# tud-airlab/mppi-isaac

Measured on AMD Instinct MI355X. Metric: MPPI control-loop Hz (K samples x H horizon), Panda 7-DoF K=4096 H=20, higher is better.
Workload: dtype f32; 1 GPU; panda_stick reach (BASELINE configs[2]): ABA from URDF, no contact, fused reach cost; K_per_gpu=4096, K_total=4096, H=20, nu=7, substeps=2, closed_loop=True, parallelism=single GPU, noise=fixed halton-spline set, sampled once at construction (outside the loop)

## Files before the change

__graft_entry__.py:

```python
import glob
import json
import os
import subprocess
import sys

ROOT = os.path.dirname(os.path.abspath(__file__))
PKG = os.path.join(ROOT, "mppi-isaac_amd")
CSRC = os.path.join(PKG, "csrc")
for p in (PKG, ROOT):
    if p not in sys.path:
        sys.path.insert(0, p)

HIPCC_FLAGS = ["--offload-arch=gfx950", "-O3", "-std=c++17", "-fPIC", "-shared",
               "-fno-slp-vectorize"]
ILP_FLAGS = ["-mllvm", "-amdgpu-sched-strategy=" + os.environ.get("MPPI_EXPERIMENT_SCHED", "max-ilp")]
if os.environ.get("MPPI_EXPERIMENT_SLP"):
    HIPCC_FLAGS.remove("-fno-slp-vectorize")


DPP_LEAD_WAIT_FROM = 9

FORESTS = [("point_robot", "point_robot")]
MOVING_FORESTS = [("jackal", "jackal")]

# ... 92 lines not shown


def _variant_jobs(variant, units, headers):
    lib = os.path.join(CSRC, f"libmppi_hip{'_' + variant if variant else ''}.so")
    objdir = os.path.join(CSRC, "build" + ("_" + variant if variant else ""))
    os.makedirs(objdir, exist_ok=True)
    flags = [f for f in HIPCC_FLAGS if f != "-shared" and not (variant == "slp" and f == "-fno-slp-vectorize")] \
        + (["-DMPPI_SECTION_CLOCKS"] if variant == "sec" else []) \
        + ([f"-DMPPI_DUP={variant[3:]}"] if variant.startswith("dup") else []) \
        + ([f"-DMPPI_PAIR_SPLIT={variant[2:]}"] if variant.startswith("ps") else []) \
        + (["-DMPPI_HWID_DEBUG"] if variant == "hwid" else []) \
        + (["-DMPPI_NO_PARK"] if variant == "nopark" else []) \
        + (["-DMPPI_CHECK"] if variant == "check" else []) \
        + ([f"-D{variant[1:].upper()}"] if variant.startswith("x") else []) \
        + (ILP_FLAGS if variant == "ilp" else []) \
        + ([f"-DMPPI_SCENE_WAVES_PER_EU={variant[1:]}"] if variant.startswith("w") and variant[1:].isdigit() else [])
    jobs = []
    for src in units:
        obj = os.path.join(objdir, os.path.basename(src) + ".o")
        if _stale(obj, [src] + headers):
            free = os.path.basename(src).startswith("topo_") and not src.endswith("_scene.hip")
            scene_flags = ["-mllvm", "-amdgpu-sched-strategy=iterative-maxocc"] if (variant == "maxocc" and not free and src.endswith("_scene.hip")) else []
            if os.environ.get("MPPI_EXPERIMENT_SCENE_SCHED") and src.endswith("_scene.hip"):
                scene_flags = ["-mllvm", "-amdgpu-sched-strategy=" + os.environ["MPPI_EXPERIMENT_SCENE_SCHED"]]
            jobs.append((src, obj, flags + (ILP_FLAGS if free and variant != "noilp" else []) + scene_flags))
    objs = [os.path.join(objdir, os.path.basename(src) + ".o") for src in units]
    return jobs, objs, lib


def build() -> None:
    from concurrent.futures import ThreadPoolExecutor
    units = [os.path.join(CSRC, "mppi_hip.hip")] + generate_sources()
    variant = os.environ.get("MPPI_BUILD_VARIANT", "")
    headers = [os.path.join(CSRC, f) for f in ("mppi_kernels.hpp", "mppi_device.hpp", "mppi_quad.hpp", "mppi_oct.hpp", "mppi_scene.hpp", "mppi_scene_quad.hpp", "mppi_scene_oct.hpp", "mppi_pack.hpp",
                                               "topologies.inc", "topo_table.inc")]
    headers.append(os.path.join(ROOT, "include", "mppi_hip.h"))
    variants = [variant] + (["check"] if variant == "" and not os.environ.get("MPPI_SKIP_CHECK_BUILD") else [])
    plans = [_variant_jobs(v, units, headers) for v in variants]
    jobs = [j for p in plans for j in p[0]]
    with ThreadPoolExecutor(max_workers=min(len(jobs), os.cpu_count() or 1) or 1) as ex:
        list(ex.map(_compile, jobs))
    hipcc = os.environ.get("HIPCC", "/opt/rocm/bin/hipcc")
    for vjobs, objs, vlib in plans:
        if vjobs or _stale(vlib, objs):
            subprocess.run([hipcc, "--offload-arch=gfx950", "-shared", "-fPIC", "-o", vlib, *objs], check=True)
    lib = plans[0][2]
    subprocess.run(["make", "-C", os.path.join(ROOT, "oracle"), "-s"], check=True)
    import mppiisaac
    from mppiisaac.backend import capi
    import ctypes
    handle = ctypes.CDLL(lib)
    for sym in capi.EXPORTED_SYMBOLS:
        getattr(handle, sym)


def smoke() -> None:
    import numpy as np
    import torch

    from mppiisaac.objectives import PandaReachObjective
    from mppiisaac.planner.mppi_isaac import MPPIisaacPlanner
    from mppiisaac.utils.config_store import load_config
    from oracle.oracle import Oracle

    assert torch.cuda.is_available(), "smoke() needs a GPU"
    cfg = load_config({"defaults": [{"mppi": "panda"}, {"isaacgym": "normal"}], "actors": ["panda_stick", "goal"],
                       "initial_actor_positions": [[0.0, 0.0, 0.0]], "nx": 14},
# ... 25 lines not shown
```

mppi-isaac_amd/csrc/mppi_hip.hip:

```cpp
#include <atomic>
#include <chrono>
#include <cstring>
#include <fstream>
#include <mutex>
#include <sstream>
#include <unordered_set>

#include <dlfcn.h>
#include <fcntl.h>
#include <spawn.h>
#include <sys/stat.h>
#include <sys/wait.h>
#include <unistd.h>

#include "mppi_kernels.hpp"
#include "topo_table.inc"

namespace {

thread_local std::string g_err;

int fail(int code, const std::string &msg) {
    g_err = msg;
    return code;
// ... 190 lines not shown
std::string lib_dir() {
    Dl_info info;
    if (dladdr((void *)&mppi_create, &info) == 0 || !info.dli_fname) return "";
    std::string p = info.dli_fname;
    const size_t k = p.rfind('/');
    return k == std::string::npos ? "." : p.substr(0, k);
}
bool file_exists(const std::string &p) {
    struct stat st;
    return stat(p.c_str(), &st) == 0 && S_ISREG(st.st_mode);
}
bool mkdir_p(const std::string &dir) {
    for (size_t i = 1; i <= dir.size(); i++)
        if (i == dir.size() || dir[i] == '/') {
            const std::string d = dir.substr(0, i);
            if (mkdir(d.c_str(), i == dir.size() ? 0700 : 0755) != 0 && errno != EEXIST) return false;
        }
    return true;
}
bool owned_and_private(const std::string &path, bool is_dir, std::string &why) {
    struct stat st;
    if (stat(path.c_str(), &st) != 0) { why = path + ": " + std::strerror(errno); return false; }
    if (is_dir ? !S_ISDIR(st.st_mode) : !S_ISREG(st.st_mode)) { why = path + " is not a " + (is_dir ? "directory" : "regular file"); return false; }
    if (st.st_uid != geteuid()) { why = path + " belongs to uid " + std::to_string((long)st.st_uid) + ", this process runs as " + std::to_string((long)geteuid()); return false; }
    if (st.st_mode & (S_IWGRP | S_IWOTH)) {
        char m[8];
        std::snprintf(m, sizeof m, "%04o", (unsigned)(st.st_mode & 07777));
        why = path + " is writable by group or others (mode " + m + ")";
        return false;
    }
    return true;
}
bool source_key(const std::string &dir, uint64_t &key, std::string &err) {
    const char *files[] = {"mppi_kernels.hpp", "mppi_device.hpp", "mppi_quad.hpp", "mppi_oct.hpp", "mppi_scene.hpp", "mppi_scene_quad.hpp", "mppi_scene_oct.hpp",
                           "mppi_pack.hpp", "topologies.inc", "../../include/mppi_hip.h"};
    uint64_t h = 1469598103934665603ull;
    for (const char *f : files) {
        std::ifstream in(dir + "/" + f, std::ios::binary);
        if (!in) { err = "kernel sources not found next to the library (" + dir + "/" + f + ")"; return false; }
        char buf[1 << 16];
        while (in.read(buf, sizeof buf) || in.gcount() > 0) {
            for (std::streamsize i = 0; i < in.gcount(); i++) h = (h ^ (unsigned char)buf[i]) * 1099511628211ull;
            if (!in) break;
        }
    }
    for (const char *f : kJitFlags)
        for (const char *q = f; *q; q++) h = (h ^ (unsigned char)*q) * 1099511628211ull;
    key = h;
    return true;
}
std::string cache_dir() {
    if (const char *e = std::getenv("MPPI_JIT_CACHE")) return e;
    if (const char *e = std::getenv("XDG_CACHE_HOME")) return std::string(e) + "/mppi_hip";
    if (const char *e = std::getenv("HOME")) return std::string(e) + "/.cache/mppi_hip";
    return "/tmp/mppi_hip_" + std::to_string((long)getuid());
}
std::string find_hipcc() {
    if (const char *e = std::getenv("HIPCC")) return e;
    for (const char *p : {"/opt/rocm/bin/hipcc", "/usr/bin/hipcc", "/usr/local/bin/hipcc"})
        if (access(p, X_OK) == 0) return p;
    return "";
}
pid_t spawn_to_log(const std::vector<std::string> &argv, const std::string &log) {
    std::vector<char *> av;
    for (const std::string &a : argv) av.push_back(const_cast<char *>(a.c_str()));
    av.push_back(nullptr);
    posix_spawn_file_actions_t fa;
// ... 193 lines not shown
                                                      (c->hm.n_light_pairs != 0 ? (size_t)kLightFloats : 0));
            c->lds_bytes_table = sizeof(unsigned) * (size_t)scene_table_dwords(c->hm.n_shapes, c->hm.n_pairs);
            const char *mode = std::getenv("MPPI_ROLLOUT");
            c->quad = !(mode && std::string(mode) == "lane");
            if (c->hm.n_bases > 1) c->quad = false;
            const bool oct = c->quad && !(mode && std::string(mode) == "quad") && cfg->num_samples >= 8;
            c->lanes_per_sample = !c->quad ? 1 : (oct ? 8 : 4);
            c->launch_rollout = c->quad ? (oct ? e->rollout_scene_oct : e->rollout_scene_quad) : e->rollout_scene;
            c->helper_wave = oct && e->rollout_scene_pair != nullptr && !(mode && std::string(mode) == "oct") && c->hm.n_pairs <= kPairKernelMaxPairs &&
                             c->hm.n_light_pairs == 0;
            if (c->helper_wave) c->launch_rollout = e->rollout_scene_pair;
            if (oct) {
                c->launch_rollout_traj = e->rollout_scene_traj;
                c->launch_materialise_traj = e->materialise_scene_traj;
            }
            c->launch_sim_step = c->quad ? e->sim_step_scene_quad : e->sim_step_scene;
            c->step_feeds_back = c->quad;
            c->launch_materialise = e->materialise_scene;
            if (hipSetDevice(device) == hipSuccess) {
                c->lds_bytes_static = e->static_lds();
                if (c->lds_bytes_quad + c->lds_bytes_table + c->lds_bytes_static <= 160 * 1024)
                    lds_err = e->raise_lds(c->lds_bytes <= 160 * 1024 ? c->lds_bytes : 0, c->lds_bytes_quad + c->lds_bytes_table);
            }
        } else {
            const char *mode = std::getenv("MPPI_ROLLOUT");
            c->quad = !(mode && std::string(mode) == "lane");
            int cus = 256;
            (void)hipDeviceGetAttribute(&cus, hipDeviceAttributeMultiprocessorCount, device);
            (void)hipGetLastError();
            const bool oct_fits = (cfg->num_samples + 7) / 8 <= 4 * cus || (mode && std::string(mode) == "oct");
            const bool oct = c->quad && !(mode && std::string(mode) == "quad") && cfg->num_samples >= 8 && oct_fits;
            c->lanes_per_sample = c->quad ? (oct ? 8 : 4) : 1;
            c->launch_rollout = c->quad ? (oct ? e->rollout_oct : e->rollout_quad) : e->rollout;
            c->launch_rollout_lane = e->rollout;
            if (c->quad) {
                c->launch_rollout_traj = oct ? e->rollout_oct_traj : e->rollout_traj;
                c->launch_materialise_traj = e->materialise_traj;
                c->launch_materialise_traj_link = e->materialise_traj_link;
            }
            c->launch_combine_world = e->combine_world;
            const char *ws = std::getenv("MPPI_WORLD_STEP");
            const bool world_quad = cfg->num_samples == 1 && !(ws && std::string(ws) == "lane");
            c->launch_sim_step = (c->quad && (cfg->num_samples >= 64 || world_quad)) ? e->sim_step_quad : e->sim_step;
            c->launch_materialise = e->materialise;
        }
        break;
    }
    if (ok && ((c->quad ? 0 : c->lds_bytes) > 160 * 1024 || c->lds_bytes_quad + c->lds_bytes_table + c->lds_bytes_static > 160 * 1024)) {
        delete c;
        return fail(MPPI_EUNSUPPORTED, "contact scene needs more than 160 KiB of LDS per workgroup (dynamic rows + table + the kernels' static __shared__)");
    }
    if (ok && lds_err != hipSuccess) {
        std::string msg = std::string("hipFuncSetAttribute(MaxDynamicSharedMemorySize): ") + hipGetErrorString(lds_err);
        delete c;
        return fail(MPPI_EHIP, msg);
    }
    if (!ok) {
        std::string t = c->topo;
        delete c;
        return fail(MPPI_EUNSUPPORTED, "kinematic tree " + t + " is not instantiated in this library and could not be built on demand: " + jit_err);
    }
    hipError_t e = hipSetDevice(device);
    if (e != hipSuccess) {
        delete c;
        return fail(MPPI_EHIP, std::string("hipSetDevice: ") + hipGetErrorString(e));
    }
// ... 690 lines not shown
#endif
int mppi_set_profiling(mppi_ctx_t *c, int on) {
    CTX_TRY(c);
    c->profiling = on != 0;
    c->profile_period = on > 1 ? on : 1;
    for (int w = 0; w < 3; w++) c->ev_used[w] = c->ev_seen[w] = 0;
    if (on)
        for (int w = 0; w < 3; w++)
            while (c->ev[w].size() < 512) {
                hipEvent_t a, b;
                if (hipEventCreate(&a) != hipSuccess || hipEventCreate(&b) != hipSuccess) { (void)hipGetLastError(); break; }
                c->ev[w].emplace_back(a, b);
            }
    return MPPI_OK;
}
int mppi_kernel_ms(mppi_ctx_t *c, int which, float *ms) {
    CTX_TRY(c);
    if (which < 0 || which > 2 || !ms) return fail(MPPI_EINVAL, "bad argument");
    HIP_TRY(hipStreamSynchronize(c->stream));
    size_t n = c->ev_used[which];
    if (n == 0) return fail(MPPI_ESTATE, "no profiled launches recorded");
    double tot = 0;
    for (size_t i = 0; i < n; i++) {
        float t = 0;
        HIP_TRY(hipEventElapsedTime(&t, c->ev[which][i].first, c->ev[which][i].second));
        tot += t;
    }
    *ms = (float)(tot / n);
    c->ev_used[which] = 0;
    return MPPI_OK;
}
int mppi_kernel_info(mppi_ctx_t *c, char *buf, int buflen) {
    CTX_TRY(c);
    std::snprintf(buf, buflen, "topology=%s rollout=%s K=%d H=%d nu=%d waves=%d block=%d bytes_alg=%zu", c->topo.c_str(), c->scene ? (c->helper_wave ? "scene-oct-pair" : (c->lanes_per_sample == 8 ? "scene-oct" : (c->quad ? "scene-quad" : "scene"))) : (c->quad ? (c->lanes_per_sample == 8 ? "oct" : "quad") : "lane"), c->K, c->H, c->nu, c->quad ? c->n_quads * ((c->lanes_per_sample == 8 && !c->scene) ? 2 : 1) : c->n_waves, kWave,
                  (size_t)4 * (3 * (size_t)c->K * c->HN + 2 * (size_t)c->K + c->HN));
    return MPPI_OK;
}

}
```

mppi-isaac_amd/csrc/mppi_kernels.hpp:

```cpp
#pragma once
#include <hip/hip_runtime.h>

#include <cstddef>
#include <cstdio>
#include <cstdlib>
#include <cstring>
#include <string>
#include <vector>

#include "mppi_pack.hpp"
#include "mppi_scene.hpp"
#include "mppi_quad.hpp"
#include "mppi_oct.hpp"
#include "mppi_scene_quad.hpp"
#include "mppi_scene_oct.hpp"

using namespace mppi;

struct mppi_ctx;

namespace {

constexpr int kWave = 64;

__device__ __forceinline__ float wave_sum(float v) {
#pragma unroll
    for (int o = 32; o > 0; o >>= 1) v += __shfl_xor(v, o, kWave);
    return v;
}
__device__ __forceinline__ float wave_min(float v) {
#pragma unroll
    for (int o = 32; o > 0; o >>= 1) v = fminf(v, __shfl_xor(v, o, kWave));
    return v;
}

template <class T>
__global__ __launch_bounds__(kWave) void k_rollout(const DevModel *__restrict__ m, const DevCfg *__restrict__ cfg,
                                                   const DevCost *__restrict__ cost, const float *__restrict__ x0_dof,
                                                   const float *__restrict__ x0_root, const float *__restrict__ U,
                                                   const float *__restrict__ eps, const float *__restrict__ prior,
                                                   float *__restrict__ du, float *__restrict__ S, float *__restrict__ viz,
                                                   float *__restrict__ partials);

__device__ __forceinline__ void wave_record(CCfg &cfg, float s, bool live, const float *__restrict__ du, int k, float *__restrict__ rec) {
    const int K = cfg.K, HN = cfg.H * cfg.nu;
    const bool fin = live && isfinite(s);
    const float beta = wave_min(fin ? s : INFINITY);
    const float w = fin ? __expf(-(s - beta) * cfg.inv_lambda) : 0.f;
    const float eta = wave_sum(w);
    const int lane = threadIdx.x & (kWave - 1);
    if (lane == 0) {
        rec[0] = beta;
        rec[1] = eta;
    }
    const size_t kk = live ? (size_t)k : 0;
    int j = 0;
// ... 313 lines not shown
        s_lin = oct_lin_place((MPPI_LDS_AS void *)s_lin_raw, &lm.b[0]);
        if ((int)threadIdx.x < T::NB) {
            DevBody b = ((const DevModel *)m)->b[threadIdx.x];
            b.k1 = oct_lin_view(b.k1);
            s_lin[threadIdx.x] = b;
        }
    }
    __syncthreads();
    const int nb = gridDim.x;
    const int chunk = (nb % 16 == 0) ? (int)(blockIdx.x % 8) * (nb / 8) + (int)(blockIdx.x / 8) : (int)blockIdx.x;
    const int k = chunk * 16 + (LAY == 8 ? (int)(threadIdx.x >> 6) * 8 + oct_slot() : (int)(threadIdx.x >> 2));
    const int lane4 = threadIdx.x & 3;
    const bool live = k < cfg->K;
    const bool leader = lane4 == 0 && (LAY == 4 || oct_half() == 0);
    float s = INFINITY;
    if (live) {
        if constexpr (LAY == 8) {
            const OctAba ab{oct_bodies(&lm.b[0], s_lin), oct_lane()};
            if (((CModel *)m)->all_revolute) s = quad_rollout<T, 0, DUMP>(lm, *(CCfg *)cfg, *(CCost *)cost, sc, x0_dof, x0_root, eps, prior, du, viz, k, leader, quad_row(), lane4 < 3, traj, ab);
            else s = quad_rollout<T, -1, DUMP>(lm, *(CCfg *)cfg, *(CCost *)cost, sc, x0_dof, x0_root, eps, prior, du, viz, k, leader, quad_row(), lane4 < 3, traj, ab);
        } else {
            if (((CModel *)m)->all_revolute) s = quad_rollout<T, 0, DUMP>(lm, *(CCfg *)cfg, *(CCost *)cost, sc, x0_dof, x0_root, eps, prior, du, viz, k, leader, quad_row(), lane4 < 3, traj);
            else s = quad_rollout<T, -1, DUMP>(lm, *(CCfg *)cfg, *(CCost *)cost, sc, x0_dof, x0_root, eps, prior, du, viz, k, leader, quad_row(), lane4 < 3, traj);
        }
        if (leader) S[k] = s;
    }
    if constexpr (LAY == 8) {
        oct_record2(*(CCfg *)cfg, s, live && leader, du, chunk * 16, partials + (size_t)chunk * (2 + cfg->H * cfg->nu), oct_slot());
        fold_after_record<2>(*(CCfg *)cfg, partials, fold_ctr, fold_out);
    } else {
        quad_record(*(CCfg *)cfg, s, live && leader, du, chunk * 16, partials + (size_t)chunk * (2 + cfg->H * cfg->nu));
        fold_after_record(*(CCfg *)cfg, partials, fold_ctr, fold_out);
    }
    if (wave_clk != nullptr && threadIdx.x == 0) {
        wave_clk[2 * chunk] = clk0;
        wave_clk[2 * chunk + 1] = wall_clock64();
    }
#endif
}

constexpr int kCombineThreads = 1024;
constexpr int kCombineGroups = 8;
constexpr int kCombineWorldThreads = 512;
template <int NT>
__device__ __forceinline__ void combine_update(CCfg &cfg, const float *__restrict__ recs, int nrec, int mode, float *__restrict__ out,
                                               float *__restrict__ U, float *__restrict__ action, float *__restrict__ beta_eta, float *s_act,
                                               const float *__restrict__ filt) {
    __shared__ float s_red[NT];
    __shared__ float s_part[kCombineGroups][MPPI_MAX_H * MPPI_MAX_NU];
    constexpr int kMaxScale = 4096;
    __shared__ float s_scale[kMaxScale];
    const int HN = cfg.H * cfg.nu, RF = 2 + HN, nu = cfg.nu;
    const int tid = threadIdx.x;
    const int wid = tid >> 6, lane = tid & 63;
    const float U_old = (mode != 0 && tid < HN) ? U[tid] : 0.f;
    const bool mine = tid < nrec;
    const float er0 = mine ? recs[(size_t)tid * RF + 1] : 0.f, br0 = mine ? recs[(size_t)tid * RF] : 0.f;
    float b = er0 > 0.f ? br0 : INFINITY;
    for (int r = tid + NT; r < nrec; r += NT)
        if (recs[(size_t)r * RF + 1] > 0.f) b = fminf(b, recs[(size_t)r * RF]);
    b = wave_min(b);
    if (lane == 0) s_red[wid] = b;
    __syncthreads();
    float beta = s_red[lane & (NT / kWave - 1)];
#pragma unroll
    for (int o = NT / kWave / 2; o > 0; o >>= 1) beta = fminf(beta, __shfl_xor(beta, o, kWave));
// ... 991 lines not shown
    const int i = threadIdx.x;
    if (i < n) {
        x0_dof[2 * i] = wq[i];
        x0_dof[2 * i + 1] = wqd[i];
    }
}

}

constexpr int kIoCmd = 16, kIoCmdSlots = 64, kIoDof = kIoCmd + 16 * kIoCmdSlots, kIoDofFloats = 32;
static_assert(kIoDofFloats == kIoMirrorRoot, "mirror layout");
constexpr int kIoFloats = kIoDof + kIoDofFloats + 13 * MPPI_MAX_ACTORS + 12;

struct mppi_ctx {
    int device = 0;
    float *h_io = nullptr, *d_io = nullptr;
    int free_slots = 2;
    unsigned io_cmd_next = 0, io_mirror_seq = 0;
    bool mirror_armed = false;
    hipStream_t stream = nullptr;
    mppi_model_t model;
    mppi_config_t cfg;
    DevModel hm;
    DevCfg hc;
    DevCost hk;
    int n = 0, A = 0, B = 0, K = 0, H = 0, nu = 0, HN = 0, RF = 0, n_waves = 0;
    int n_quads = 0;
    int lanes_per_sample = 1;
    float *d_traj = nullptr;
    DevCost *d_cost_none = nullptr;
    void (*launch_rollout_traj)(mppi_ctx *) = nullptr;
    void (*launch_materialise_traj)(mppi_ctx *, float *, float *, float *, float *) = nullptr;
    void (*launch_materialise_traj_link)(mppi_ctx *, int, float *) = nullptr;
    bool helper_wave = false;
    int n_partials = 0;
    bool quad = false;
    DevModel *d_model = nullptr;
    DevCfg *d_cfg = nullptr;
    DevCost *d_cost = nullptr;
    float *d_x0_dof = nullptr, *d_x0_root = nullptr, *d_U = nullptr, *d_eps = nullptr, *d_du = nullptr, *d_S = nullptr;
    float *d_prior = nullptr, *d_viz = nullptr, *d_partials = nullptr, *d_record = nullptr, *d_action = nullptr, *d_beta_eta = nullptr;
    float *d_q = nullptr, *d_qd = nullptr, *d_ctrl = nullptr;
    float *d_base = nullptr, *d_fr = nullptr, *d_cf = nullptr;
    float *d_filter = nullptr;
    float *h_action = nullptr;
    unsigned *d_seq = nullptr;
    unsigned seq_expected = 0;
    bool use_filter = false;
    bool scene = false;
    size_t lds_bytes = 0, lds_bytes_quad = 0;
    size_t lds_bytes_table = 0;
    size_t lds_bytes_static = 0;
    double *d_basis = nullptr, *d_sigma = nullptr;
    const float *eps_in = nullptr;
    bool has_prior = false, has_cost = false, profiling = false;
    bool partials_valid = false;
    bool fold = false;
    unsigned *d_fold_ctr = nullptr;
    float *d_fold = nullptr, *fold_out = nullptr;
    const float *recs_cur = nullptr;
    unsigned long long *d_wave_clk = nullptr;
    bool wave_clk_on = false;
    std::vector<std::pair<hipEvent_t, hipEvent_t>> ev[3];
    size_t ev_used[3] = {0, 0, 0}, ev_seen[3] = {0, 0, 0};
    int profile_period = 1;
    void (*launch_rollout)(mppi_ctx *) = nullptr;
    void (*launch_rollout_lane)(mppi_ctx *) = nullptr;
    bool prog_lane = false;
    void (*launch_sim_step)(mppi_ctx *, int, int, const float *) = nullptr;
    void (*launch_materialise)(mppi_ctx *, float *, float *, float *, float *) = nullptr;
    void (*launch_combine_world)(mppi_ctx *, const float *, int, mppi_ctx *) = nullptr;
    void (*launch_eval_cost)(mppi_ctx *, int, const float *, const float *, const float *, const float *, float *) = nullptr;
    std::string topo;
    float *fb_dof = nullptr, *fb_root = nullptr;
    bool step_feeds_back = false;
    void *d_inbox = nullptr;
    void **d_peers = nullptr;
    std::vector<void *> h_peers, ipc_opened;
    int mb_rank = -1, mb_n = 0, mb_nrec = 0;
    unsigned *d_mb_seq = nullptr, *d_mb_status = nullptr;
    float *d_gathered = nullptr, *d_own_rec = nullptr;
    size_t inbox_bytes = 0;
    bool peers_dirty = false;
    bool inbox_fine = false;
};

namespace mppi {
struct TopoEntry {
    int nb;
    int parents[MPPI_MAX_BODIES];
    size_t scene_lds_floats;
    int free_slots;
    void (*rollout)(mppi_ctx *);
    void (*rollout_quad)(mppi_ctx *);
    void (*rollout_oct)(mppi_ctx *);
    void (*rollout_oct_traj)(mppi_ctx *);
    void (*rollout_scene)(mppi_ctx *);
    void (*rollout_scene_quad)(mppi_ctx *);
    void (*rollout_scene_oct)(mppi_ctx *);
    void (*rollout_scene_pair)(mppi_ctx *);
    void (*rollout_traj)(mppi_ctx *);
    void (*rollout_scene_traj)(mppi_ctx *);
    void (*materialise_traj)(mppi_ctx *, float *, float *, float *, float *);
    void (*materialise_traj_link)(mppi_ctx *, int, float *);
    void (*materialise_scene_traj)(mppi_ctx *, float *, float *, float *, float *);
    void (*sim_step)(mppi_ctx *, int, int, const float *);
    void (*sim_step_quad)(mppi_ctx *, int, int, const float *);
    void (*sim_step_scene)(mppi_ctx *, int, int, const float *);
    void (*sim_step_scene_quad)(mppi_ctx *, int, int, const float *);
    void (*materialise)(mppi_ctx *, float *, float *, float *, float *);
    void (*materialise_scene)(mppi_ctx *, float *, float *, float *, float *);
    void (*combine_world)(mppi_ctx *, const float *, int, mppi_ctx *);
    void (*eval_cost)(mppi_ctx *, int, const float *, const float *, const float *, const float *, float *);
    hipError_t (*raise_lds)(size_t, size_t);
    size_t (*static_lds)();
};
}

namespace {

template <class T>
void launch_rollout_scene_t(mppi_ctx *c) {
    hipLaunchKernelGGL(k_rollout_scene<T>, dim3(c->n_waves), dim3(kWave), c->lds_bytes, c->stream, c->d_model, c->d_cfg, c->d_cost, c->d_x0_dof,
                       c->d_x0_root, c->d_U, c->eps_in, c->has_prior ? c->d_prior : nullptr, c->d_du, c->d_S, c->cfg.want_rollouts ? c->d_viz : nullptr,
                       c->d_partials);
}
template <class T>
constexpr bool kHasOctSolve = (T::NB > 4);
inline bool scene_oct_solve(const mppi_ctx *c) {
// ... 106 lines not shown
    auto ask = [&](const void *f) {
        hipFuncAttributes a;
        if (hipFuncGetAttributes(&a, f) == hipSuccess && a.sharedSizeBytes > mx) mx = a.sharedSizeBytes;
        else (void)hipGetLastError();
    };
    ask(reinterpret_cast<const void *>(&k_rollout_scene_quad<T, 4>));
    ask(reinterpret_cast<const void *>(&k_rollout_scene_quad<T, 8>));
    ask(reinterpret_cast<const void *>(&k_rollout_scene_quad<T, 8, 1, true>));
    if constexpr (kHasOctSolve<T>) {
        ask(reinterpret_cast<const void *>(&k_rollout_scene_quad<T, 8, 1, false, true>));
        ask(reinterpret_cast<const void *>(&k_rollout_scene_quad<T, 8, 1, true, true>));
    }
    if constexpr (T::NB <= 4) {
        ask(reinterpret_cast<const void *>(&k_rollout_scene_quad<T, 8, 2>));
        ask(reinterpret_cast<const void *>(&k_rollout_scene_quad<T, 8, 2, true>));
    }
    ask(reinterpret_cast<const void *>(&k_sim_step_scene_quad<T>));
    return mx;
}

template <class T>
void launch_rollout_quad_t(mppi_ctx *c) {
    hipLaunchKernelGGL(k_rollout_quad<T>, dim3(c->n_quads), dim3(kWave), 0, c->stream, c->d_model, c->d_cfg, c->d_cost, c->d_x0_dof, c->d_x0_root,
                       c->d_U, c->eps_in, c->has_prior ? c->d_prior : nullptr, c->d_du, c->d_S, c->cfg.want_rollouts ? c->d_viz : nullptr, c->d_partials,
                       c->fold ? c->d_fold_ctr : nullptr, c->fold_out, c->wave_clk_on ? c->d_wave_clk : nullptr);
}
template <class T>
void launch_rollout_oct_t(mppi_ctx *c) {
    hipLaunchKernelGGL((k_rollout_quad<T, false, 8>), dim3(c->n_quads), dim3(2 * kWave), 0, c->stream, c->d_model, c->d_cfg, c->d_cost, c->d_x0_dof, c->d_x0_root,
                       c->d_U, c->eps_in, c->has_prior ? c->d_prior : nullptr, c->d_du, c->d_S, c->cfg.want_rollouts ? c->d_viz : nullptr, c->d_partials,
                       c->fold ? c->d_fold_ctr : nullptr, c->fold_out, c->wave_clk_on ? c->d_wave_clk : nullptr);
}
template <class T>
void launch_rollout_oct_traj_t(mppi_ctx *c) {
    hipLaunchKernelGGL((k_rollout_quad<T, true, 8>), dim3(c->n_quads), dim3(2 * kWave), 0, c->stream, c->d_model, c->d_cfg, c->d_cost_none, c->d_x0_dof, c->d_x0_root,
                       c->d_U, c->eps_in, c->has_prior ? c->d_prior : nullptr, c->d_du, c->d_S, (float *)nullptr, c->d_partials,
                       (unsigned *)nullptr, c->fold_out, (unsigned long long *)nullptr, c->d_traj);
}
template <class T>
void launch_rollout_traj_t(mppi_ctx *c) {
    hipLaunchKernelGGL((k_rollout_quad<T, true>), dim3(c->n_quads), dim3(kWave), 0, c->stream, c->d_model, c->d_cfg, c->d_cost_none, c->d_x0_dof, c->d_x0_root,
                       c->d_U, c->eps_in, c->has_prior ? c->d_prior : nullptr, c->d_du, c->d_S, (float *)nullptr, c->d_partials,
                       (unsigned *)nullptr, c->fold_out, (unsigned long long *)nullptr, c->d_traj);
}
template <class T>
void launch_materialise_traj_t(mppi_ctx *c, float *dof, float *root, float *rb, float *cf) {
    const size_t HK = (size_t)c->H * c->K;
    hipLaunchKernelGGL(k_materialise<T>, dim3((unsigned)((HK + kWave - 1) / kWave)), dim3(kWave), 0, c->stream, c->d_model, (int)HK, c->d_x0_root, c->d_traj,
                       c->d_traj + (size_t)T::NB * HK, dof, root, rb, cf);
}
template <class T>
void launch_materialise_traj_link_t(mppi_ctx *c, int link, float *out) {
    const size_t HK = (size_t)c->H * c->K;
    hipLaunchKernelGGL(k_materialise_link<T>, dim3((unsigned)((HK + kWave - 1) / kWave)), dim3(kWave), 0, c->stream, c->d_model, (int)HK, c->d_x0_root, c->d_traj,
                       c->d_traj + (size_t)T::NB * HK, link, out);
}
template <class T>
void launch_combine_world_t(mppi_ctx *p, const float *recs, int n, mppi_ctx *w) {
    MailboxArgs mb;
    if (recs == nullptr) {
        mb.wave_recs = p->recs_cur; mb.n_wave = p->n_partials; mb.own = p->d_own_rec; mb.RF = p->RF; mb.rank = p->mb_rank; mb.n = p->mb_n;
        mb.peers = (void *const *)p->d_peers; mb.seq_ctr = p->d_mb_seq; mb.inbox = p->d_inbox; mb.gathered = p->d_gathered; mb.status = p->d_mb_status;
        mb.max_ticks = 200000000ull;
    }
    hipLaunchKernelGGL(k_combine_world<T>, dim3(1), dim3(kCombineWorldThreads), 0, p->stream, p->d_cfg, recs, n, p->d_U, p->d_action, p->d_beta_eta,
                       w->d_model, w->d_x0_root, w->d_q, w->d_qd, p->d_x0_dof, p->use_filter ? p->d_filter : nullptr, mb);
// ... 1 lines not shown
template <class T>
void launch_eval_cost_t(mppi_ctx *c, int n, const float *dof, const float *root, const float *rb, const float *cf, float *out) {
    hipLaunchKernelGGL(k_eval_cost<T>, dim3((n + kWave - 1) / kWave), dim3(kWave), 0, c->stream, c->d_model, c->d_cost, n, dof, root, rb, cf, out);
}
template <class T>
void launch_rollout_t(mppi_ctx *c) {
    hipLaunchKernelGGL(k_rollout<T>, dim3(c->n_waves), dim3(kWave), 0, c->stream, c->d_model, c->d_cfg, c->d_cost, c->d_x0_dof, c->d_x0_root,
                       c->d_U, c->eps_in, c->has_prior ? c->d_prior : nullptr, c->d_du, c->d_S, c->cfg.want_rollouts ? c->d_viz : nullptr, c->d_partials);
}
template <class T>
void launch_sim_step_t(mppi_ctx *c, int mode, int t, const float *u_ext) {
    hipLaunchKernelGGL(k_sim_step<T>, dim3(c->n_waves), dim3(kWave), 0, c->stream, c->d_model, c->d_cfg, mode, t, u_ext, c->d_x0_root, c->d_U,
                       c->eps_in, c->has_prior ? c->d_prior : nullptr, c->d_du, c->d_ctrl, c->d_q, c->d_qd);
}
template <class T>
void launch_sim_step_quad_t(mppi_ctx *c, int mode, int t, const float *u_ext) {
    hipLaunchKernelGGL(k_sim_step_quad<T>, dim3((c->K + 15) / 16), dim3(kWave), 0, c->stream, c->d_model, c->d_cfg, mode, t, u_ext, c->d_x0_root, c->d_U,
                       c->eps_in, c->has_prior ? c->d_prior : nullptr, c->d_du, c->d_ctrl, c->d_q, c->d_qd);
}
template <class T>
void launch_materialise_t(mppi_ctx *c, float *dof, float *root, float *rb, float *cf) {
    hipLaunchKernelGGL(k_materialise<T>, dim3(c->n_waves), dim3(kWave), 0, c->stream, c->d_model, c->K, c->d_x0_root, c->d_q, c->d_qd, dof, root,
                       rb, cf, c->mirror_armed ? c->d_io + kIoDof : nullptr, reinterpret_cast<unsigned *>(c->d_io), c->io_mirror_seq);
}

template <class T>
void fill_topo_entry_free(TopoEntry &e) {
    e.nb = T::NB;
    for (int i = 0; i < T::NB; i++) e.parents[i] = T::par[i];
    e.rollout = &launch_rollout_t<T>;
    e.rollout_quad = &launch_rollout_quad_t<T>;
    e.rollout_oct = &launch_rollout_oct_t<T>;
    e.rollout_oct_traj = &launch_rollout_oct_traj_t<T>;
    e.sim_step = &launch_sim_step_t<T>;
    e.sim_step_quad = &launch_sim_step_quad_t<T>;
    e.rollout_traj = &launch_rollout_traj_t<T>;
    e.materialise_traj = &launch_materialise_traj_t<T>;
    e.materialise_traj_link = &launch_materialise_traj_link_t<T>;
    e.materialise = &launch_materialise_t<T>;
    e.combine_world = &launch_combine_world_t<T>;
    e.eval_cost = &launch_eval_cost_t<T>;
}
template <class T>
void fill_topo_entry_scene(TopoEntry &e) {
    e.scene_lds_floats = (size_t)SceneLayout<T>::kCf;
    e.free_slots = kFreeSlots;
    e.rollout_scene = &launch_rollout_scene_t<T>;
    e.rollout_scene_quad = &launch_rollout_scene_quad_t<T, 4>;
    e.rollout_scene_oct = &launch_rollout_scene_quad_t<T, 8>;
    e.rollout_scene_pair = T::NB <= 4 ? &launch_rollout_scene_pair_t<T> : nullptr;
    e.sim_step_scene = &launch_sim_step_scene_t<T>;
    e.sim_step_scene_quad = &launch_sim_step_scene_quad_t<T>;
    e.rollout_scene_traj = &launch_rollout_scene_traj_t<T>;
    e.materialise_scene_traj = &launch_materialise_scene_traj_t<T>;
    e.materialise_scene = &launch_materialise_scene_t<T>;
    e.raise_lds = &raise_lds_limit<T>;
    e.static_lds = &static_lds_bytes_scene<T>;
}

}
```

mppi-isaac_amd/csrc/mppi_quad.hpp:

```cpp
#pragma once
#include <cstddef>

#include "mppi_device.hpp"

namespace mppi {

#if defined(__HIP_DEVICE_COMPILE__)
typedef float QF;
template <int CTRL>
__device__ __forceinline__ float quad_dpp(float x) {
    return __builtin_bit_cast(float, __builtin_amdgcn_mov_dpp(__builtin_bit_cast(int, x), CTRL, 0xf, 0xf, true));
}
__device__ __forceinline__ QF rot1(QF x) { return quad_dpp<0x49>(x); }
__device__ __forceinline__ QF rot2(QF x) { return quad_dpp<0x92>(x); }
template <int K>
__device__ __forceinline__ QF bc(QF x) { return quad_dpp<K * 0x55>(x); }
__device__ __forceinline__ int quad_row() { int l = threadIdx.x & 3; return l == 3 ? 0 : l; }
__device__ __forceinline__ QF qsel(float x0, float x1, float x2) { int r = quad_row(); return r == 0 ? x0 : (r == 1 ? x1 : x2); }
__device__ __forceinline__ QF qrep(float x) { return x; }
__device__ __forceinline__ float qlane0(QF x) { return x; }
__device__ __forceinline__ QF qsqrt(QF x) { return __builtin_amdgcn_sqrtf(x); }
__device__ __forceinline__ QF qrcp(QF x) { float r = __builtin_amdgcn_rcpf(x); return r * (2.f - x * r); }
__device__ __forceinline__ QF qabs(QF x) { return fabsf(x); }
__device__ __forceinline__ QF qclamp(QF v, QF lo, QF hi) { return __builtin_amdgcn_fmed3f(v, lo, hi); }
// ... 622 lines not shown
            {
                const QF lo = qrep(blk0[i].lower), hi = qrep(blk0[i].upper), z = qrep(0.f);
                const QF vlo = qclamp((lo - q[i]) * inv_h, qrep(-b.vmax), z), vhi = qclamp((hi - q[i]) * inv_h, z, qrep(b.vmax));
                v = qclamp(v, vlo, vhi);
                x = qclamp(q[i] + h * v, lo, hi);
            }
            q[i] = x;
            qd[i] = v;
        });
        quad_fk_from<T, JT>(blk0, q, P);
    }
}

template <class T, int JT, int LO, int HI>
MPPI_HD void quad_body_pose(const QPose<T, JT> &P, int body, QM3 &Rb, QF &pb) {
    if constexpr (HI - LO == 1) {
        if constexpr (LO < 0) {
            Rb = P.rot_base();
            pb = P.pos_base();
        } else {
            Rb = P.rot(LO);
            pb = P.pos(LO);
        }
#if defined(__HIP_DEVICE_COMPILE__)
        asm volatile("");
#endif
    } else {
        constexpr int MID = LO + (HI - LO) / 2;
        if (body < MID) quad_body_pose<T, JT, LO, MID>(P, body, Rb, pb);
        else quad_body_pose<T, JT, MID, HI>(P, body, Rb, pb);
    }
}

template <class T, class M, int JT>
MPPI_HD void quad_link_pose(M &m, const QPose<T, JT> &P, int l, QM3 &R, QF &p) {
    auto &L = m.l[l];
#if defined(__HIP_DEVICE_COMPILE__)
    const int body = __builtin_amdgcn_readfirstlane(L.body);
#else
    const int body = L.body;
#endif
    QM3 Rb;
    QF pb;
    quad_body_pose<T, JT, -1, T::NB>(P, body < 0 ? -1 : (body < T::NB ? body : T::NB - 1), Rb, pb);
    for (int c = 0; c < 3; c++) R.c[c] = Rb.c[0] * L.R[c] + Rb.c[1] * L.R[3 + c] + Rb.c[2] * L.R[6 + c];
    p = pb + Rb.c[0] * L.p[0] + Rb.c[1] * L.p[1] + Rb.c[2] * L.p[2];
}

struct StepConsts {
    CtrlBlock u_min, u_max, inv_sigma;
    float goal[4];
    float w[4];
    CtrlBlock Urow[MPPI_MAX_H];
};
#if defined(__HIP_DEVICE_COMPILE__)
typedef const MPPI_LDS_AS StepConsts LStep;
#else
typedef const StepConsts LStep;
#endif
MPPI_HD float step_const_entry(CCfg &cfg, CCost &c, const float *root, const float *U, int j) {
    constexpr int kU = (int)(offsetof(StepConsts, Urow) / sizeof(float));
    if (j < 16) return cfg.u_min.v[j];
    if (j < 32) return cfg.u_max.v[j - 16];
    if (j < 48) return cfg.inv_sigma.v[j - 32];
    if (j < 52) {
        const int a = c.actor[0], i = j - 48;
        if (i == 3) return 0.f;
        if (a >= 0) return root[13 * a + i];
        return i < 2 ? c.w[1 + i] : 0.f;
    }
    if (j < 56) return c.w[j - 52];
    const int t = (j - kU) >> 4, col = (j - kU) & 15;
    return (t < cfg.H && col < cfg.nu) ? U[t * cfg.nu + col] : 0.f;
}
MPPI_HD int step_const_count(CCfg &cfg) { return (int)(offsetof(StepConsts, Urow) / sizeof(float)) + cfg.H * 16; }

template <class T>
MPPI_HD QF quad_stage_cost(int kind, LStep &sc, const QF *q, const QM3 &R, QF p) {
    if (kind == kCostPointReach) {
// ... 139 lines not shown
```

Measured before the change: 8204 Hz (4096-sample x 20-step control iterations per second, summed over GPUs).

## Add oct-pair rollout splitting dynamics and control/cost work across wave pairs

Adds a new free-space rollout kernel in which each 256-thread block runs two owner waves that integrate dynamics and two helper waves that compute controls, noise application and stage costs. The two sides exchange per-step control rows and link poses through LDS with double-buffered slots and named barriers, and the weighted reduction is done over 16 samples per block. The host selects this kernel when the oct path applies, H<=32 and K/16 fits within the CU count. The aim is to take control and cost arithmetic off the critical dynamics path so it runs concurrently. In exchange it adds per-step barrier synchronisation and LDS traffic, and uses more waves per sample.

Result: faster. 9466 Hz (4096-sample x 20-step control iterations per second, summed over GPUs), median of 6 (+15.4%).

```diff
diff --git a/__graft_entry__.py b/__graft_entry__.py
--- a/__graft_entry__.py
+++ b/__graft_entry__.py
@@ -148,7 +148,7 @@
     from concurrent.futures import ThreadPoolExecutor
     units = [os.path.join(CSRC, "mppi_hip.hip")] + generate_sources()
     variant = os.environ.get("MPPI_BUILD_VARIANT", "")
-    headers = [os.path.join(CSRC, f) for f in ("mppi_kernels.hpp", "mppi_device.hpp", "mppi_quad.hpp", "mppi_oct.hpp", "mppi_scene.hpp", "mppi_scene_quad.hpp", "mppi_scene_oct.hpp", "mppi_pack.hpp",
+    headers = [os.path.join(CSRC, f) for f in ("mppi_kernels.hpp", "mppi_device.hpp", "mppi_quad.hpp", "mppi_oct.hpp", "mppi_oct_pair.hpp", "mppi_scene.hpp", "mppi_scene_quad.hpp", "mppi_scene_oct.hpp", "mppi_pack.hpp",
                                                "topologies.inc", "topo_table.inc")]
     headers.append(os.path.join(ROOT, "include", "mppi_hip.h"))
     variants = [variant] + (["check"] if variant == "" and not os.environ.get("MPPI_SKIP_CHECK_BUILD") else [])
diff --git a/mppi-isaac_amd/csrc/mppi_hip.hip b/mppi-isaac_amd/csrc/mppi_hip.hip
--- a/mppi-isaac_amd/csrc/mppi_hip.hip
+++ b/mppi-isaac_amd/csrc/mppi_hip.hip
@@ -246,7 +246,7 @@
     return true;
 }
 bool source_key(const std::string &dir, uint64_t &key, std::string &err) {
-    const char *files[] = {"mppi_kernels.hpp", "mppi_device.hpp", "mppi_quad.hpp", "mppi_oct.hpp", "mppi_scene.hpp", "mppi_scene_quad.hpp", "mppi_scene_oct.hpp",
+    const char *files[] = {"mppi_kernels.hpp", "mppi_device.hpp", "mppi_quad.hpp", "mppi_oct.hpp", "mppi_oct_pair.hpp", "mppi_scene.hpp", "mppi_scene_quad.hpp", "mppi_scene_oct.hpp",
                            "mppi_pack.hpp", "topologies.inc", "../../include/mppi_hip.h"};
     uint64_t h = 1469598103934665603ull;
     for (const char *f : files) {
@@ -506,6 +506,10 @@
             const bool oct = c->quad && !(mode && std::string(mode) == "quad") && cfg->num_samples >= 8 && oct_fits;
             c->lanes_per_sample = c->quad ? (oct ? 8 : 4) : 1;
             c->launch_rollout = c->quad ? (oct ? e->rollout_oct : e->rollout_quad) : e->rollout;
+            const bool pair_forced = mode && std::string(mode) == "oct-pair";
+            c->pair_free = oct && e->rollout_oct_pair != nullptr && !(mode && std::string(mode) == "oct") && cfg->horizon <= kPairTableH &&
+                           ((cfg->num_samples + 15) / 16 <= cus || pair_forced);
+            if (c->pair_free) c->launch_rollout = e->rollout_oct_pair;
             c->launch_rollout_lane = e->rollout;
             if (c->quad) {
                 c->launch_rollout_traj = oct ? e->rollout_oct_traj : e->rollout_traj;
@@ -1262,7 +1266,7 @@
 }
 int mppi_kernel_info(mppi_ctx_t *c, char *buf, int buflen) {
     CTX_TRY(c);
-    std::snprintf(buf, buflen, "topology=%s rollout=%s K=%d H=%d nu=%d waves=%d block=%d bytes_alg=%zu", c->topo.c_str(), c->scene ? (c->helper_wave ? "scene-oct-pair" : (c->lanes_per_sample == 8 ? "scene-oct" : (c->quad ? "scene-quad" : "scene"))) : (c->quad ? (c->lanes_per_sample == 8 ? "oct" : "quad") : "lane"), c->K, c->H, c->nu, c->quad ? c->n_quads * ((c->lanes_per_sample == 8 && !c->scene) ? 2 : 1) : c->n_waves, kWave,
+    std::snprintf(buf, buflen, "topology=%s rollout=%s K=%d H=%d nu=%d waves=%d block=%d bytes_alg=%zu", c->topo.c_str(), c->scene ? (c->helper_wave ? "scene-oct-pair" : (c->lanes_per_sample == 8 ? "scene-oct" : (c->quad ? "scene-quad" : "scene"))) : (c->quad ? (c->lanes_per_sample == 8 ? (c->pair_free ? "oct-pair" : "oct") : "quad") : "lane"), c->K, c->H, c->nu, c->quad ? c->n_quads * ((c->lanes_per_sample == 8 && !c->scene) ? (c->pair_free ? 4 : 2) : 1) : c->n_waves, kWave,
                   (size_t)4 * (3 * (size_t)c->K * c->HN + 2 * (size_t)c->K + c->HN));
     return MPPI_OK;
 }
diff --git a/mppi-isaac_amd/csrc/mppi_kernels.hpp b/mppi-isaac_amd/csrc/mppi_kernels.hpp
--- a/mppi-isaac_amd/csrc/mppi_kernels.hpp
+++ b/mppi-isaac_amd/csrc/mppi_kernels.hpp
@@ -12,6 +12,7 @@
 #include "mppi_scene.hpp"
 #include "mppi_quad.hpp"
 #include "mppi_oct.hpp"
+#include "mppi_oct_pair.hpp"
 #include "mppi_scene_quad.hpp"
 #include "mppi_scene_oct.hpp"
 
@@ -22,6 +23,7 @@
 namespace {
 
 constexpr int kWave = 64;
+constexpr int kPairTableH = 32;
 
 __device__ __forceinline__ float wave_sum(float v) {
 #pragma unroll
@@ -401,6 +403,152 @@
         quad_record(*(CCfg *)cfg, s, live && leader, du, chunk * 16, partials + (size_t)chunk * (2 + cfg->H * cfg->nu));
         fold_after_record(*(CCfg *)cfg, partials, fold_ctr, fold_out);
     }
+    if (wave_clk != nullptr && threadIdx.x == 0) {
+        wave_clk[2 * chunk] = clk0;
+        wave_clk[2 * chunk + 1] = wall_clock64();
+    }
+#endif
+}
+
+#if defined(__HIP_DEVICE_COMPILE__)
+template <class T>
+__device__ __forceinline__ void oct_record_pair(CCfg &cfg, LStep &sc, float s, bool live_leader, bool helper, const MPPI_LDS_AS float *utab, int k0,
+                                                float *__restrict__ rec, int slot) {
+    constexpr int NT = 4 * kWave, SPG = 16, kStride = PairLayout<T>::kStride, kRow = PairLayout<T>::kRow;
+    __shared__ float s_w[SPG], s_b[2], s_e[2];
+    const int K = cfg.K, nu = cfg.nu, HN = cfg.H * nu;
+    const int lane = threadIdx.x & (kWave - 1), wv = (threadIdx.x >> 6) & 1;
+    const bool fin = live_leader && isfinite(s);
+    const float bw = wave_min(fin ? s : INFINITY);
+    if (helper && lane == 0) s_b[wv] = bw;
+    MPPI_BARRIER(12);
+    const float beta = fminf(s_b[0], s_b[1]);
+    const float w = fin ? __expf(-(s - beta) * cfg.inv_lambda) : 0.f;
+    const float ew = wave_sum(w);
+    if (helper && lane == 0) s_e[wv] = ew;
+    if (helper && (lane & 3) == 0 && ((lane >> 3) & 1) == 0) s_w[wv * 8 + slot] = w;
+    MPPI_BARRIER(13);
+    if (threadIdx.x == 0) {
+        rec[0] = beta;
+        rec[1] = s_e[0] + s_e[1];
+    }
+    const int nlive = K - k0 < SPG ? K - k0 : SPG;
+    if (nlive == SPG && (K & 3) == 0) {
+        constexpr int kTrips = 2, NR = 2 * kWave;
+        if (threadIdx.x >= NR) return;
+        float wq[SPG];
+#pragma unroll
+        for (int q = 0; q < SPG; q++) wq[q] = s_w[q];
+        for (int j0 = threadIdx.x; j0 < HN; j0 += kTrips * NR) {
+            float4 v[kTrips][SPG / 4];
+#pragma unroll
+            for (int t = 0; t < kTrips; t++) {
+                const int j = j0 + t * NR;
+                if (j < HN) {
+                    const int ts = j / nu, c = j - ts * nu;
+                    const float Ut = sc.Urow[ts].v[c];
+                    const MPPI_LDS_AS float *col = utab + ts * kRow + c;
+#pragma unroll
+                    for (int q = 0; q < SPG / 4; q++)
+                        v[t][q] = make_float4(col[(4 * q) * kStride] - Ut, col[(4 * q + 1) * kStride] - Ut, col[(4 * q + 2) * kStride] - Ut, col[(4 * q + 3) * kStride] - Ut);
+                }
+            }
+#pragma unroll
+            for (int t = 0; t < kTrips; t++) {
+                const int j = j0 + t * NR;
+                if (j < HN) {
+                    float acc = 0.f;
+#pragma unroll
+                    for (int q = 0; q < SPG / 4; q++)
+                        acc += v[t][q].x * wq[4 * q] + v[t][q].y * wq[4 * q + 1] + v[t][q].z * wq[4 * q + 2] + v[t][q].w * wq[4 * q + 3];
+                    rec[2 + j] = acc;
+                }
+            }
+        }
+        return;
+    }
+    for (int j = threadIdx.x; j < HN; j += NT) {
+        const int t = j / nu, c = j - t * nu;
+        const float Ut = sc.Urow[t].v[c];
+        const MPPI_LDS_AS float *col = utab + t * kRow + c;
+        float acc = 0.f;
+        for (int q = 0; q < nlive; q++) acc += (col[q * kStride] - Ut) * s_w[q];
+        rec[2 + j] = acc;
+    }
+}
+
+#endif
+
+template <class T>
+__global__ __launch_bounds__(4 * kWave) void k_rollout_oct_pair(const DevModel *__restrict__ m, const DevCfg *__restrict__ cfg,
+                                                                const DevCost *__restrict__ cost, const float *__restrict__ x0_dof,
+                                                                const float *__restrict__ x0_root, const float *__restrict__ U,
+                                                                const float *__restrict__ eps, const float *__restrict__ prior,
+                                                                float *__restrict__ du, float *__restrict__ S, float *__restrict__ viz,
+                                                                float *__restrict__ partials, unsigned *__restrict__ fold_ctr, float *__restrict__ fold_out,
+                                                                unsigned long long *__restrict__ wave_clk) {
+#if defined(__HIP_DEVICE_COMPILE__)
+    const unsigned long long clk0 = wave_clk != nullptr ? wall_clock64() : 0ull;
+    asm volatile("; one wavefront per SIMD" ::: "a31");
+    constexpr int NT = 4 * kWave;
+    constexpr int kModelBytes = (int)((offsetof(DevModel, fr) + 15) / 16 * 16);
+    __shared__ __attribute__((aligned(64))) uint4 s_model[kModelBytes / 16];
+    constexpr int kModelTrips = (kModelBytes / 16 + NT - 1) / NT;
+    uint4 mv[kModelTrips];
+#pragma unroll
+    for (int it = 0; it < kModelTrips; it++) {
+        const int i = (int)threadIdx.x + it * NT;
+        mv[it] = reinterpret_cast<const uint4 *>(m)[i < kModelBytes / 16 ? i : 0];
+    }
+    __shared__ __attribute__((aligned(64))) float s_step[sizeof(StepConsts) / sizeof(float)];
+    {
+        const int n = step_const_count(*(CCfg *)cfg);
+        for (int j = threadIdx.x; j < n; j += NT) s_step[j] = step_const_entry(*(CCfg *)cfg, *(CCost *)cost, x0_root, U, j);
+    }
+#pragma unroll
+    for (int it = 0; it < kModelTrips; it++) {
+        const int i = (int)threadIdx.x + it * NT;
+        if (i < kModelBytes / 16) s_model[i] = mv[it];
+    }
+    __shared__ __attribute__((aligned(256))) uint4 s_lin_raw[oct_lin_raw_bytes(T::NB) / 16];
+    LModel &lm = *(LModel *)s_model;
+    LStep &sc = *(LStep *)s_step;
+    MPPI_LDS_AS DevBody *s_lin = oct_lin_place((MPPI_LDS_AS void *)s_lin_raw, &lm.b[0]);
+    if ((int)threadIdx.x < T::NB) {
+        DevBody b = ((const DevModel *)m)->b[threadIdx.x];
+        b.k1 = oct_lin_view(b.k1);
+        s_lin[threadIdx.x] = b;
+    }
+    static_assert(kPairTableH == kPairMaxH, "the host selects by the table the kernel allocates");
+    __shared__ __attribute__((aligned(16))) float s_utab[PairLayout<T>::kTable];
+    __shared__ f32x4 s_xa[2 * 2 * kWave], s_xb[2 * 2 * kWave];
+    __syncthreads();
+    const int nb = gridDim.x;
+    const int chunk = (nb % 16 == 0) ? (int)(blockIdx.x % 8) * (nb / 8) + (int)(blockIdx.x / 8) : (int)blockIdx.x;
+    const int wave = (int)(threadIdx.x >> 6), own = wave & 1;
+    const bool helper = wave >= 2;
+    const int lane = threadIdx.x & (kWave - 1);
+    const int k = chunk * 16 + own * 8 + oct_slot();
+    const int K = cfg->K;
+    const bool live = k < K;
+    const int ke = live ? k : K - 1;
+    const bool leader = (threadIdx.x & 3) == 0 && oct_half() == 0;
+    const bool want_viz = cfg->want_rollouts && viz != nullptr;
+    MPPI_LDS_AS float *utab = (MPPI_LDS_AS float *)s_utab;
+    MPPI_LDS_AS float *urow = utab + (own * 8 + oct_slot()) * PairLayout<T>::kStride;
+    LF4 *xa = (LF4 *)s_xa + own * kWave + lane, *xb = (LF4 *)s_xb + own * kWave + lane;
+    float s = INFINITY;
+    if (!helper) {
+        const OctAba ab{oct_bodies(&lm.b[0], s_lin), oct_lane()};
+        if (((CModel *)m)->all_revolute) pair_owner<T, 0>(lm, *(CCfg *)cfg, *(CCost *)cost, x0_dof, x0_root, urow, xa, xb, 2 * kWave, want_viz, ab);
+        else pair_owner<T, -1>(lm, *(CCfg *)cfg, *(CCost *)cost, x0_dof, x0_root, urow, xa, xb, 2 * kWave, want_viz, ab);
+    } else {
+        s = pair_helper<T>(lm, *(CCfg *)cfg, *(CCost *)cost, sc, eps, prior, du, viz, ke, quad_row(), urow, xa, xb, 2 * kWave);
+        if (!live) s = INFINITY;
+        if (live && leader) S[k] = s;
+    }
+    oct_record_pair<T>(*(CCfg *)cfg, sc, s, helper && live && leader, helper, utab, chunk * 16, partials + (size_t)chunk * (2 + cfg->H * cfg->nu), oct_slot());
+    fold_after_record<4>(*(CCfg *)cfg, partials, fold_ctr, fold_out);
     if (wave_clk != nullptr && threadIdx.x == 0) {
         wave_clk[2 * chunk] = clk0;
         wave_clk[2 * chunk + 1] = wall_clock64();
@@ -1458,6 +1606,7 @@
     void (*launch_rollout_traj)(mppi_ctx *) = nullptr;
     void (*launch_materialise_traj)(mppi_ctx *, float *, float *, float *, float *) = nullptr;
     void (*launch_materialise_traj_link)(mppi_ctx *, int, float *) = nullptr;
+    bool pair_free = false;
     bool helper_wave = false;
     int n_partials = 0;
     bool quad = false;
@@ -1521,6 +1670,7 @@
     void (*rollout_quad)(mppi_ctx *);
     void (*rollout_oct)(mppi_ctx *);
     void (*rollout_oct_traj)(mppi_ctx *);
+    void (*rollout_oct_pair)(mppi_ctx *);
     void (*rollout_scene)(mppi_ctx *);
     void (*rollout_scene_quad)(mppi_ctx *);
     void (*rollout_scene_oct)(mppi_ctx *);
@@ -1693,6 +1843,12 @@
                        c->fold ? c->d_fold_ctr : nullptr, c->fold_out, c->wave_clk_on ? c->d_wave_clk : nullptr);
 }
 template <class T>
+void launch_rollout_oct_pair_t(mppi_ctx *c) {
+    hipLaunchKernelGGL(k_rollout_oct_pair<T>, dim3(c->n_quads), dim3(4 * kWave), 0, c->stream, c->d_model, c->d_cfg, c->d_cost, c->d_x0_dof, c->d_x0_root,
+                       c->d_U, c->eps_in, c->has_prior ? c->d_prior : nullptr, c->d_du, c->d_S, c->cfg.want_rollouts ? c->d_viz : nullptr, c->d_partials,
+                       c->fold ? c->d_fold_ctr : nullptr, c->fold_out, c->wave_clk_on ? c->d_wave_clk : nullptr);
+}
+template <class T>
 void launch_rollout_oct_traj_t(mppi_ctx *c) {
     hipLaunchKernelGGL((k_rollout_quad<T, true, 8>), dim3(c->n_quads), dim3(2 * kWave), 0, c->stream, c->d_model, c->d_cfg, c->d_cost_none, c->d_x0_dof, c->d_x0_root,
                        c->d_U, c->eps_in, c->has_prior ? c->d_prior : nullptr, c->d_du, c->d_S, (float *)nullptr, c->d_partials,
@@ -1760,6 +1916,7 @@
     e.rollout_quad = &launch_rollout_quad_t<T>;
     e.rollout_oct = &launch_rollout_oct_t<T>;
     e.rollout_oct_traj = &launch_rollout_oct_traj_t<T>;
+    e.rollout_oct_pair = &launch_rollout_oct_pair_t<T>;
     e.sim_step = &launch_sim_step_t<T>;
     e.sim_step_quad = &launch_sim_step_quad_t<T>;
     e.rollout_traj = &launch_rollout_traj_t<T>;
diff --git a/mppi-isaac_amd/csrc/mppi_oct_pair.hpp b/mppi-isaac_amd/csrc/mppi_oct_pair.hpp
--- /dev/null
+++ b/mppi-isaac_amd/csrc/mppi_oct_pair.hpp
@@ -0,0 +1,151 @@
+#pragma once
+#include "mppi_oct.hpp"
+#include "mppi_quad.hpp"
+
+namespace mppi {
+
+#if defined(__HIP_DEVICE_COMPILE__)
+constexpr int kPairMaxH = 32;
+template <class T>
+struct PairLayout {
+    static constexpr int MAXC = T::NB < kMaxNu ? T::NB : kMaxNu;
+    static constexpr int kStride = (MAXC + 3) & ~3;
+    static constexpr int kRow = 16 * kStride;
+    static constexpr int kTable = kPairMaxH * kRow;
+};
+typedef float f32x4 __attribute__((ext_vector_type(4)));
+typedef MPPI_LDS_AS f32x4 LF4;
+
+template <class T, int JT, class M, class AB>
+__device__ __forceinline__ void pair_owner(M &m0, CCfg &cfg0, CCost &cost0, const float *dof0, const float *root, const MPPI_LDS_AS float *urow, LF4 *xa,
+                                           LF4 *xb, int xslot, bool want_viz, const AB &ab) {
+    constexpr int NB = T::NB, MAXC = PairLayout<T>::MAXC, kStride = PairLayout<T>::kStride, kRow = PairLayout<T>::kRow;
+    const int H = cfg0.H, kind = cost0.kind, link = cost0.link[0], viz_link = cfg0.viz_link;
+    const bool cmd_identity = m0.cmd_identity != 0, need_link = kind == kCostPandaReach, point = kind == kCostPointReach;
+    const bool own_viz = want_viz && (viz_link != link || !need_link);
+    QF q[NB], qd[NB], target[NB];
+    static_for<0, NB>([&](auto ic) MPPI_LAMBDA {
+        constexpr int i = ic;
+        q[i] = qrep(dof0[2 * i]);
+        qd[i] = qrep(dof0[2 * i + 1]);
+    });
+    QPose<T, JT> P;
+    quad_base<T>(m0, root, P);
+    quad_fk<T>(m0, q, P);
+    M *mp = &m0;
+    MPPI_BARRIER(10);
+    for (int t = 0; t < H; t++) {
+        float u[kMaxNu];
+#pragma unroll
+        for (int c = MAXC; c < kMaxNu; c++) u[c] = 0.f;
+#pragma unroll
+        for (int j = 0; j < kStride / 4; j++) {
+            const f32x4 v = *reinterpret_cast<const LF4 *>(urow + t * kRow + 4 * j);
+#pragma unroll
+            for (int c = 0; c < 4; c++)
+                if (4 * j + c < MAXC) u[4 * j + c] = v[c];
+        }
+        if (cmd_identity) {
+            static_for<0, NB>([&](auto ic) MPPI_LAMBDA { target[ic] = qrep(u[ic < kMaxNu ? (int)ic : 0]); });
+        } else {
+            M &m = *launder(mp);
+            static_for<0, NB>([&](auto ic) MPPI_LAMBDA {
+                constexpr int i = ic;
+                const CmdBlock b = load_block<CmdBlock>(m.b[i].cmd);
+                float tg = 0.f;
+#pragma unroll
+                for (int c = 0; c < MAXC; c++) tg += b.v[c] * u[c];
+                target[i] = qrep(tg);
+            });
+        }
+        quad_step<T>(*mp, P, q, qd, target, ab);
+        const int s = (t & 1) * xslot;
+        if (need_link) {
+            QM3 Rb;
+            QF pb;
+            quad_link_body_pose<T>(*launder(mp), P, link, Rb, pb);
+            xa[s] = f32x4{Rb.c[0], Rb.c[1], Rb.c[2], pb};
+        } else if (point) {
+            xa[s] = f32x4{q[0], q[NB > 1 ? 1 : 0], 0.f, 0.f};
+        }
+        if (own_viz) {
+            QM3 Rb;
+            QF pb;
+            quad_link_body_pose<T>(*launder(mp), P, viz_link, Rb, pb);
+            xb[s] = f32x4{Rb.c[0], Rb.c[1], Rb.c[2], pb};
+        }
+        asm volatile("s_waitcnt lgkmcnt(0)" ::: "memory");
+        MPPI_BARRIER(11);
+    }
+}
+
+template <class T, class M>
+__device__ __forceinline__ QF pair_helper(M &m0, CCfg &cfg0, CCost &cost0, LStep &sc, const float *eps, const float *prior, float *du, float *viz, int k,
+                                          int row, MPPI_LDS_AS float *urow, const LF4 *xa, const LF4 *xb, int xslot) {
+    constexpr int MAXC = PairLayout<T>::MAXC, kStride = PairLayout<T>::kStride, kRow = PairLayout<T>::kRow;
+    const int K = cfg0.K, nu = cfg0.nu, H = cfg0.H, kind = cost0.kind, link = cost0.link[0], viz_link = cfg0.viz_link;
+    const float lambda = cfg0.lambda, gamma = cfg0.gamma;
+    const bool abs_cost = cfg0.noise_abs_cost != 0, want_viz = cfg0.want_rollouts && viz != nullptr;
+    const bool need_link = kind == kCostPandaReach;
+    const bool own_viz = want_viz && (viz_link != link || !need_link);
+    const int g = cfg0.k_offset + k;
+    const bool is_null = cfg0.sample_null_action && g == cfg0.k_total - 1;
+    const bool is_prior = cfg0.use_priors && prior != nullptr && g == cfg0.k_total - 2;
+    ControlRows<MAXC> rows;
+    load_controls_q<MAXC>(sc, eps, prior, nu, K, 0, k, rows);
+    const bool special_here = __builtin_amdgcn_ballot_w64(is_null || is_prior) != 0;
+    const bool plain_controls = !special_here && nu == MAXC && !abs_cost;
+    float ctrl = 0.f, disc = 1.f;
+    QF S = qrep(0.f);
+    auto controls = [&](int t) MPPI_LAMBDA {
+        float u[kMaxNu];
+        ctrl += plain_controls ? apply_controls_q<MAXC, true>(sc, lambda, abs_cost, nu, K, rows, t, k, is_null, is_prior, false, du, u)
+                               : apply_controls_q<MAXC, false>(sc, lambda, abs_cost, nu, K, rows, t, k, is_null, is_prior, false, du, u);
+#pragma unroll
+        for (int j = 0; j < kStride / 4; j++) {
+            f32x4 v;
+#pragma unroll
+            for (int c = 0; c < 4; c++) v[c] = 4 * j + c < MAXC ? u[4 * j + c] : 0.f;
+            *reinterpret_cast<LF4 *>(urow + t * kRow + 4 * j) = v;
+        }
+        load_controls_q<MAXC>(sc, eps, prior, nu, K, t + 1 < H ? t + 1 : t, k, rows);
+    };
+    controls(0);
+    asm volatile("s_waitcnt lgkmcnt(0)" ::: "memory");
+    MPPI_BARRIER(10);
+    if (H > 1) controls(1);
+    M *mp = &m0;
+    for (int t = 0; t < H; t++) {
+        asm volatile("s_waitcnt lgkmcnt(0)" ::: "memory");
+        MPPI_BARRIER(11);
+        if (t + 2 < H) controls(t + 2);
+        const int s = (t & 1) * xslot;
+        QM3 Rl;
+        QF pl = qrep(0.f);
+        for (int c = 0; c < 3; c++) Rl.c[c] = qrep(0.f);
+        QF q[2] = {qrep(0.f), qrep(0.f)};
+        if (need_link) {
+            const f32x4 a = xa[s];
+            quad_link_from_body(launder(mp)->l[link], QM3{{a[0], a[1], a[2]}}, a[3], Rl, pl);
+        } else if (kind == kCostPointReach) {
+            const f32x4 a = xa[s];
+            q[0] = a[0];
+            q[1] = a[1];
+        }
+        S += disc * quad_stage_cost<T>(kind, sc, q, Rl, pl);
+        disc *= gamma;
+        if (want_viz) {
+            QM3 R;
+            QF p = pl;
+            if (own_viz) {
+                const f32x4 b = xb[s];
+                quad_link_from_body(launder(mp)->l[viz_link], QM3{{b[0], b[1], b[2]}}, b[3], R, p);
+            }
+            viz[((unsigned)(t * 3 + row)) * (unsigned)K + (unsigned)k] = p;
+        }
+    }
+    return S + ctrl;
+}
+#endif
+
+}
diff --git a/mppi-isaac_amd/csrc/mppi_quad.hpp b/mppi-isaac_amd/csrc/mppi_quad.hpp
--- a/mppi-isaac_amd/csrc/mppi_quad.hpp
+++ b/mppi-isaac_amd/csrc/mppi_quad.hpp
@@ -678,19 +678,26 @@
     }
 }
 
+template <class LK>
+MPPI_HD void quad_link_from_body(LK &L, const QM3 &Rb, QF pb, QM3 &R, QF &p) {
+    for (int c = 0; c < 3; c++) R.c[c] = Rb.c[0] * L.R[c] + Rb.c[1] * L.R[3 + c] + Rb.c[2] * L.R[6 + c];
+    p = pb + Rb.c[0] * L.p[0] + Rb.c[1] * L.p[1] + Rb.c[2] * L.p[2];
+}
+template <class T, class M, int JT>
+MPPI_HD void quad_link_body_pose(M &m, const QPose<T, JT> &P, int l, QM3 &Rb, QF &pb) {
+#if defined(__HIP_DEVICE_COMPILE__)
+    const int body = __builtin_amdgcn_readfirstlane(m.l[l].body);
+#else
+    const int body = m.l[l].body;
+#endif
+    quad_body_pose<T, JT, -1, T::NB>(P, body < 0 ? -1 : (body < T::NB ? body : T::NB - 1), Rb, pb);
+}
 template <class T, class M, int JT>
 MPPI_HD void quad_link_pose(M &m, const QPose<T, JT> &P, int l, QM3 &R, QF &p) {
-    auto &L = m.l[l];
-#if defined(__HIP_DEVICE_COMPILE__)
-    const int body = __builtin_amdgcn_readfirstlane(L.body);
-#else
-    const int body = L.body;
-#endif
     QM3 Rb;
     QF pb;
-    quad_body_pose<T, JT, -1, T::NB>(P, body < 0 ? -1 : (body < T::NB ? body : T::NB - 1), Rb, pb);
-    for (int c = 0; c < 3; c++) R.c[c] = Rb.c[0] * L.R[c] + Rb.c[1] * L.R[3 + c] + Rb.c[2] * L.R[6 + c];
-    p = pb + Rb.c[0] * L.p[0] + Rb.c[1] * L.p[1] + Rb.c[2] * L.p[2];
+    quad_link_body_pose<T>(m, P, l, Rb, pb);
+    quad_link_from_body(m.l[l], Rb, pb, R, p);
 }
 
 struct StepConsts {
```
